# voletiv/mcvd-pytorch

Hardware: NVIDIA H100
Metric: frames/sec @100 DDPM steps, SMMNIST 64x64 (higher is better)
Workload: dtype f32 (fp16 hi/lo split on wgmma, fp32 accumulate)

## Files before the change

mcvd_b200/csrc/conv_umma.cu:

```cuda
#include <cuda.h>
#include <cuda_fp16.h>

#include <algorithm>
#include <cstring>

#include "mcvd_common.cuh"
#include "umma_ptx.cuh"

namespace mcvd {

constexpr int STAT_MT = 128;

namespace {

using namespace ptx;

constexpr int NPROD = 96;
constexpr int W_LOAD = 3;
constexpr int W_CONS = 4;
constexpr int NT_MAX3 = 192;
constexpr int REG_PROD3 = 96, REG_CONS3 = 136;
constexpr float STAT_SCALE = 65536.0f;
constexpr int TAB_NB = 8;
constexpr int HP_MAX = 512;
constexpr int PPT = (HP_MAX + NPROD - 1) / NPROD;
constexpr int RAW_STAGES = 2;
constexpr int MAX_RESIDENT = 12;

struct ConvMaps {
  CUtensorMap src[4];
  CUtensorMap tab;
};

struct ConvArgs {
  const float* s0;
  const float* s1;
  const float* s2;
  const float* s3;
  int C2, C3, nKB0;
  const __half* wpk;
  const float* bias;
  const float* res;
  const float* tab;
  int tab_planar;
  float* dst;
  unsigned long long* stats;
  int NJ;
  int B, H, W, C0, C1, Cout;
  int ks;
  int Wp, Pimg;
  int Qtot;
  int KB;
  int HP;
  int boxn, nbox;
  int raw_off, raw_stage, tab_off;
  int RA;
  int halo0;
  int nKB;
  int NB;
  int SA;
  int NPI;
  int tiles_n, ntiles;
  int act_in, act_out;
  int split;
  int tab_nb;
  float wscale, oscale;
};

__device__ __forceinline__ int decode_pos(const ConvArgs& a, int q, int& b_out) {
  if (q < 0 || q >= a.Qtot) return -1;
  const int b = q / a.Pimg;
  const int r = q - b * a.Pimg;
  const int rr = r / a.Wp, cc = r - rr * a.Wp;
  b_out = b;
  if (a.ks == 3) {
    if (rr == 0 || cc == 0) return -1;
    return (b * a.H + (rr - 1)) * a.W + (cc - 1);
  }
  return (b * a.H + rr) * a.W + cc;
}

__device__ __forceinline__ int first_raw(const ConvArgs& a, int q) {
  q = max(q, 0);
  if (q >= a.Qtot) return a.B * a.H * a.W;
  if (a.ks == 1) return q;
  const int b = q / a.Pimg;
  const int r = q - b * a.Pimg;
  const int rr = r / a.Wp, cc = r - rr * a.Wp;
  if (rr == 0) return b * a.H * a.W;
  return (b * a.H + (rr - 1)) * a.W + (cc == 0 ? 0 : cc - 1);
}

template <int NT, int NWG>
__global__ void __launch_bounds__(128 * (NWG + 1), 1) k_conv_umma(const ConvArgs a,
                                                                  const __grid_constant__ ConvMaps maps) {
  static_assert(NWG == 2 || (NWG == 3 && NT <= NT_MAX3), "three consumer warpgroups hold at most 96 accumulators");
  constexpr int MT = 64 * NWG;
  constexpr int NTHREADS = 128 * (NWG + 1);
  constexpr int NCONS = 4 * NWG;
  extern __shared__ __align__(1024) uint8_t smem_raw[];
  const int chunks = a.KB / 8;
  const uint32_t a_half_bytes = (uint32_t)chunks * a.HP * 16;
  const uint32_t a_stage_bytes = 2 * a_half_bytes;
  constexpr uint32_t b_step_bytes = 64u * NT;
  const uint32_t b_stage_bytes = (uint32_t)(a.KB / 16) * b_step_bytes;
  uint8_t* a_base = smem_raw;
  uint8_t* b_base = a_base + (size_t)a.SA * a_stage_bytes;
  uint8_t* raw_base = smem_raw + a.raw_off;
  int* pinfo = reinterpret_cast<int*>(raw_base + (size_t)a.RA * a.raw_stage);
  unsigned long long* stat_s = reinterpret_cast<unsigned long long*>(pinfo + PPT * NPROD);
  uint64_t* bars = reinterpret_cast<uint64_t*>(stat_s + (a.stats ? a.NJ * 2 * NT : 0));
  const uint32_t bar0 = smem_u32(bars);
  auto A_FULL = [&](int i) { return bar0 + 8u * i; };
  auto A_EMPTY = [&](int i) { return bar0 + 8u * (a.SA + i); };
  auto B_FULL = [&](int i) { return bar0 + 8u * (2 * a.SA + i); };
  auto B_EMPTY = [&](int i) { return bar0 + 8u * (2 * a.SA + a.NB + i); };
  auto R_FULL = [&](int i) { return bar0 + 8u * (2 * a.SA + 2 * a.NB + i); };
  const int groups_n = a.tiles_n / a.NPI;

  const int tid = threadIdx.x, warp = tid >> 5, lane = tid & 31;
  const int taps = a.ks * a.ks;

  if (tid == 0) {
    for (int i = 0; i < a.SA; ++i) { mbar_init(A_FULL(i), NPROD); mbar_init(A_EMPTY(i), NCONS); }
    for (int i = 0; i < a.NB; ++i) { mbar_init(B_FULL(i), 1); mbar_init(B_EMPTY(i), NCONS); }
    for (int i = 0; i < a.RA; ++i) mbar_init(R_FULL(i), 1);
    fence_barrier_init();
  }
  if (a.stats)
    for (int i = tid; i < a.NJ * 2 * NT; i += NTHREADS) stat_s[i] = 0ull;
  __syncthreads();

  if (warp < W_CONS) {
    if constexpr (NWG == 3) setmaxnreg_dec<REG_PROD3>();
    if (warp < W_LOAD) {
      const bool has_tab = a.tab != nullptr;
      const int ch = (lane >> 3) % chunks;
      const int ppass = NPROD / chunks;
      const int pp = warp * (32 / chunks) + (lane & 7) + 8 * ((lane >> 3) / chunks);
      const uint32_t rowb = (uint32_t)a.KB * 4, smask = a.KB == 32 ? 7u : 3u;
      auto tile_b0_of = [&](int t) {
        const int q_first = (t / groups_n) * MT - a.halo0;
        return q_first <= 0 ? 0 : min(a.B - 1, q_first / a.Pimg);
      };
      const uint32_t raw0 = smem_u32(raw_base);
      const uint32_t main_bytes = (uint32_t)a.nbox * a.boxn * rowb, ctr_bytes = (uint32_t)MT * rowb;
      const uint32_t tab_bytes = (uint32_t)a.tab_nb * a.KB * (a.tab_planar ? 12 : 16);
      int it = blockIdx.x, ikb = 0, ig = 0;
      auto issue_next = [&]() {
        if (it >= a.ntiles) return;
        const int p0 = (it / groups_n) * MT;
        const bool seg2 = ikb >= a.nKB0;
        int si, cc0;
        if (!seg2) {
          const int c0 = ikb * a.KB;
          if (c0 < a.C0) { si = 0; cc0 = c0; } else { si = 1; cc0 = c0 - a.C0; }
        } else {
          const int c0 = (ikb - a.nKB0) * a.KB;
          if (c0 < a.C2) { si = 2; cc0 = c0; } else { si = 3; cc0 = c0 - a.C2; }
        }
        const bool use_tab = has_tab && !seg2;
        const uint32_t dst = raw0 + (uint32_t)(ig % a.RA) * a.raw_stage;
        const uint32_t bar = R_FULL(ig % a.RA);
        mbar_arrive_expect_tx(bar, (seg2 ? ctr_bytes : main_bytes) + (use_tab ? tab_bytes : 0u));
        if (seg2) {
          tma_load_2d(dst, &maps.src[si], cc0, first_raw(a, p0), bar);
        } else {
          const int r0 = first_raw(a, p0 - a.halo0);
          for (int i = 0; i < a.nbox; ++i)
            tma_load_2d(dst + (uint32_t)i * a.boxn * rowb, &maps.src[si], cc0, r0 + i * a.boxn, bar);
        }
        if (use_tab) {
          if (a.tab_planar) tma_load_3d(dst + a.tab_off, &maps.tab, ikb * a.KB, 0, tile_b0_of(it), bar);
          else tma_load_2d(dst + a.tab_off, &maps.tab, 4 * ikb * a.KB, tile_b0_of(it), bar);
        }
        ++ig;
        if (++ikb == a.nKB) { ikb = 0; it += gridDim.x; }
      };
      if (tid == 0)
        for (int i = 0; i < a.RA - 1; ++i) issue_next();
      int g = 0;
      for (int t = blockIdx.x; t < a.ntiles; t += gridDim.x) {
        const int p0 = (t / groups_n) * MT;
        const int tb0 = tile_b0_of(t);
        const int raw_m = first_raw(a, p0 - a.halo0), raw_c = first_raw(a, p0);
        named_bar_sync(1, NPROD);
        for (int h = tid; h < a.HP; h += NPROD) {
          int b = tb0;
          const int pix = decode_pos(a, p0 - a.halo0 + h, b);
          pinfo[h] = pix < 0 ? -1 : ((b - tb0) << 16) | (pix - raw_m);
        }
        for (int kb = 0; kb < a.nKB; ++kb, ++g) {
          const int st = g % a.SA;
          const bool seg2 = kb >= a.nKB0;
          const bool use_tab = has_tab && !seg2;
          const int h_lo = seg2 ? a.halo0 : 0, h_hi = seg2 ? a.halo0 + MT : a.HP;
          const int roff = seg2 ? raw_c - raw_m : 0;
          named_bar_sync(1, NPROD);
          if (tid == 0) issue_next();
// ... 55 lines not shown
              hv = make_uint4(hw[0], hw[1], hw[2], hw[3]);
              lv = make_uint4(lw[0], lw[1], lw[2], lw[3]);
            }
            *reinterpret_cast<uint4*>(hi_base + (size_t)h * 16) = hv;
            *reinterpret_cast<uint4*>(lo_base + (size_t)h * 16) = lv;
          }
          fence_proxy_async();
          mbar_arrive(A_FULL(st));
        }
      }
    } else if (warp == W_LOAD) {
      if (elect_one()) {
        const uint32_t b0 = smem_u32(b_base);
        const int per_tile = a.nKB0 * taps + (a.nKB - a.nKB0);
        int st = 0, ph = 1;
        for (int t = blockIdx.x; t < a.ntiles; t += gridDim.x)
         for (int j = 0; j < a.NPI; ++j) {
          const int nt = (t % groups_n) * a.NPI + j;
          const uint8_t* wsrc = reinterpret_cast<const uint8_t*>(a.wpk) + (size_t)nt * per_tile * b_stage_bytes;
          for (int i = 0; i < per_tile; ++i) {
            mbar_wait(B_EMPTY(st), ph);
            mbar_arrive_expect_tx(B_FULL(st), b_stage_bytes);
            bulk_g2s(b0 + (uint32_t)st * b_stage_bytes, wsrc + (size_t)i * b_stage_bytes, b_stage_bytes, B_FULL(st));
            if (++st == a.NB) { st = 0; ph ^= 1; }
          }
        }
      }
      __syncwarp();
    }
  } else {
    if constexpr (NWG == 3) setmaxnreg_inc<REG_CONS3>();
    const int wg = (warp - W_CONS) >> 2;
    const int wq = (warp - W_CONS) & 3;
    const int ksteps = a.KB / 16;
    const uint32_t a_lbo = (uint32_t)a.HP * 16;
    const uint64_t a_proto = make_desc(0, a_lbo, 128), b_proto = make_desc(0, NT * 16, 128);
    const uint32_t a_half16 = a_half_bytes >> 4, b_lo16 = 2u * NT;
    const uint32_t a0_16 = smem_u32(a_base) >> 4, b0_16 = smem_u32(b_base) >> 4;
    const uint32_t a_stage16 = a_stage_bytes >> 4, b_stage16 = b_stage_bytes >> 4;
    const uint32_t a_lbo16 = a_lbo >> 4;
    int bst = 0, bph = 0, g0 = 0;
    for (int t = blockIdx.x; t < a.ntiles; t += gridDim.x, g0 += a.nKB)
     for (int j = 0; j < a.NPI; ++j) {
      const int p0 = (t / groups_n) * MT;
      const int n0 = ((t % groups_n) * a.NPI + j) * NT;
      const bool last_n = j == a.NPI - 1;
      float acc[NT / 2];
#pragma unroll
      for (int i = 0; i < NT / 2; ++i) acc[i] = 0.f;
      int pend_b = -1, pend_a = -1;
      for (int kb = 0; kb < a.nKB; ++kb) {
        const int g = g0 + kb;
        const int st = g % a.SA;
        mbar_wait(A_FULL(st), (g / a.SA) & 1);
        const uint32_t a_hi16 = a0_16 + (uint32_t)st * a_stage16 + (uint32_t)(a.halo0 + 64 * wg);
        const int ntap = (kb < a.nKB0) ? taps : 1;
        for (int tap = 0; tap < ntap; ++tap) {
          mbar_wait(B_FULL(bst), bph);
          const int shift = (a.ks == 3 && kb < a.nKB0) ? ((tap / 3 - 1) * a.Wp + (tap % 3 - 1)) : 0;
          const uint32_t a_tap16 = a_hi16 + (uint32_t)shift;
// ... 13 lines not shown
          wgmma_wait<1>();
          if (pend_b >= 0 && lane == 0) mbar_arrive(B_EMPTY(pend_b));
          if (pend_a >= 0 && lane == 0) mbar_arrive(A_EMPTY(pend_a));
          pend_b = bst;
          pend_a = (tap == ntap - 1 && last_n) ? st : -1;
          if (++bst == a.NB) { bst = 0; bph ^= 1; }
        }
      }
      wgmma_wait<0>();
#pragma unroll
      for (int i = 0; i < NT / 2; ++i) reg_fence(acc[i]);
      if (lane == 0) { mbar_arrive(B_EMPTY(pend_b)); if (pend_a >= 0) mbar_arrive(A_EMPTY(pend_a)); }

      const int r0 = 64 * wg + 16 * wq + (lane >> 2);
      const int cq = 2 * (lane & 3);
      int pix[2], slot[2];
      const int tile_b0 = min(a.B - 1, p0 / a.Pimg);
#pragma unroll
      for (int i = 0; i < 2; ++i) {
        int b = 0;
        pix[i] = decode_pos(a, p0 + r0 + 8 * i, b);
        slot[i] = pix[i] >= 0 ? b - tile_b0 : -1;
      }
      unsigned jmask = 0;
      if (a.stats) {
#pragma unroll 1
        for (int jj = 0; jj < a.NJ; ++jj)
          if (__ballot_sync(0xffffffffu, slot[0] == jj || slot[1] == jj)) jmask |= 1u << jj;
      }
#pragma unroll
      for (int j = 0; j < NT / 8; ++j) {
        const int n = n0 + 8 * j + cq;
        const float2 bv = a.bias ? __ldg(reinterpret_cast<const float2*>(a.bias + n)) : make_float2(0.f, 0.f);
        float v[2][2];
#pragma unroll
        for (int i = 0; i < 2; ++i) {
          float2 rv = make_float2(0.f, 0.f);
          if (a.res && pix[i] >= 0) rv = __ldg(reinterpret_cast<const float2*>(a.res + (long long)pix[i] * a.Cout + n));
          float x0 = (acc[4 * j + 2 * i] * a.wscale + bv.x + rv.x) * a.oscale;
          float x1 = (acc[4 * j + 2 * i + 1] * a.wscale + bv.y + rv.y) * a.oscale;
          if (a.act_out) { x0 = silu_f(x0); x1 = silu_f(x1); }
          v[i][0] = x0; v[i][1] = x1;
          if (pix[i] >= 0) *reinterpret_cast<float2*>(a.dst + (long long)pix[i] * a.Cout + n) = make_float2(x0, x1);
        }
        if (a.stats) {
#pragma unroll 1
          for (int jj = 0; jj < a.NJ; ++jj) {
            if (!(jmask & (1u << jj))) continue;
#pragma unroll
            for (int e = 0; e < 2; ++e) {
              long long s1 = 0;
              unsigned long long s2 = 0;
#pragma unroll
              for (int i = 0; i < 2; ++i) {
                if (slot[i] == jj) {
                  const int xi = __float2int_rn(v[i][e] * STAT_SCALE);
                  s1 += xi;
                  s2 += (unsigned long long)((long long)xi * (long long)xi);
                }
              }
#pragma unroll
              for (int o = 4; o <= 16; o <<= 1) {
                s1 += __shfl_xor_sync(0xffffffffu, s1, o);
                s2 += __shfl_xor_sync(0xffffffffu, s2, o);
              }
              if (lane < 4) {
                unsigned long long* sp = stat_s + (size_t)jj * 2 * NT + 8 * j + cq + e;
                atomicAdd(sp, (unsigned long long)s1);
                atomicAdd(sp + NT, s2);
              }
            }
          }
        }
      }
      if (a.stats) {
        named_bar_sync(2, 32 * NCONS);
        const int et = tid - W_CONS * 32;
        unsigned long long* gp = a.stats + (size_t)(p0 / MT) * a.NJ * 2 * a.Cout;
        for (int i = et; i < a.NJ * 2 * NT; i += 32 * NCONS) {
          const int jp = i / NT, n = i - jp * NT;
          gp[(size_t)jp * a.Cout + n0 + n] = stat_s[i];
          stat_s[i] = 0ull;
        }
        named_bar_sync(2, 32 * NCONS);
      }
    }
  }
}

__global__ void k_pack_weights(const float* __restrict__ w, __half* __restrict__ out, int taps, int Cin, int Cout,
                               int NT, int KB, float scale, int stage_off, int per_unit) {
  const int ksteps = KB / 16, nKB = Cin / KB, nNT = Cout / NT;
  const long long total = (long long)nNT * nKB * taps * ksteps * 2 * NT * 8;
  for (long long i = (long long)blockIdx.x * blockDim.x + threadIdx.x; i < total;
       i += (long long)gridDim.x * blockDim.x) {
    int e = (int)(i % 8);
    long long t = i / 8;
    int n = (int)(t % NT); t /= NT;
    int j = (int)(t % 2); t /= 2;
// ... 24 lines not shown
  if (C2 + C3 > 0 && pick_kb(C2, C3) < kb) kb = pick_kb(C2, C3);
  return kb;
}

struct Plan {
  int HP, NB, NJ;
  int boxn, nbox, tab_nb;
  int raw_off, raw_stage, tab_off, RA;
  size_t smem;
};

constexpr size_t SMEM_LIMIT = 227 * 1024;

size_t round1024(size_t x) { return (x + 1023) & ~(size_t)1023; }

bool make_plan(int H, int W, int ks, int KB, int NT, bool stats, int SA, int MT, Plan& p) {
  const int Wp = ks == 3 ? W + 1 : W;
  const int Pimg = ks == 3 ? (H + 1) * (W + 1) : H * W;
  const int halo0 = ks == 3 ? Wp + 1 : 0;
  p.HP = (MT + 2 * halo0 + 7) & ~7;
  p.NJ = (MT - 1) / Pimg + 2;
  if (p.HP > HP_MAX) return false;
  p.nbox = p.HP > 256 ? 2 : 1;
  p.boxn = p.nbox == 1 ? p.HP : ((p.HP / 2 + 7) & ~7);
  p.tab_nb = std::min(p.HP / Pimg + 2, TAB_NB);
  p.tab_off = p.nbox * p.boxn * KB * 4;
  p.raw_stage = (int)round1024((size_t)p.tab_off + (size_t)p.tab_nb * KB * 16);
  const size_t a_stage = (size_t)2 * (KB / 8) * p.HP * 16;
  const size_t b_stage = (size_t)(KB / 16) * 64 * NT;
  const size_t stat_bytes = stats ? (size_t)p.NJ * 2 * NT * 8 : 0;
  const size_t pinfo_bytes = (size_t)PPT * NPROD * 4;
  size_t bar_bytes = 0, fixed = 0;
  for (p.RA = RAW_STAGES; p.RA >= 1; --p.RA) {
    bar_bytes = 8 * (2 * SA + 20 + p.RA);
    fixed = round1024(SA * a_stage) + (size_t)p.RA * p.raw_stage + pinfo_bytes + stat_bytes + bar_bytes;
    if (fixed + 2 * b_stage <= SMEM_LIMIT) break;
  }
  if (p.RA == 0) return false;
  p.NB = (int)((SMEM_LIMIT - fixed) / b_stage);
  if (p.NB > 10) p.NB = 10;
  p.raw_off = (int)round1024(SA * a_stage + (size_t)p.NB * b_stage);
  p.smem = (size_t)p.raw_off + (size_t)p.RA * p.raw_stage + pinfo_bytes + stat_bytes + bar_bytes;
  return p.smem <= SMEM_LIMIT;
}

// ... 46 lines not shown
    if (nwg == 3) return launch_nt<NT, 3>(a, m, smem, grid, s);
  return launch_nt<NT, 2>(a, m, smem, grid, s);
}

int launch_conv(const McvdOp& op, cudaStream_t s, bool planar) {
  const char* name = planar ? "CONV_UMMA2" : "CONV_UMMA";
  MCVD_CHECK(op.src0 && op.w && op.dst && (op.C1 == 0 || op.src1), "%s: null pointer", name);
  MCVD_CHECK(op.i0 == 1 || op.i0 == 3, "%s: kernel size %d unsupported", name, op.i0);
  ConvArgs a;
  a.s0 = (const float*)op.src0; a.s1 = (const float*)op.src1; a.wpk = (const __half*)op.w;
  a.s2 = (const float*)op.src2; a.s3 = (const float*)op.src3; a.C2 = op.src2 ? op.C2 : 0; a.C3 = op.src3 ? op.C3 : 0;
  a.bias = (const float*)op.bias; a.res = (const float*)op.aux0; a.tab = (const float*)op.aux1;
  a.tab_planar = planar ? 1 : 0;
  a.dst = (float*)op.dst;
  a.stats = (unsigned long long*)op.dst2;
  a.B = op.B; a.H = op.H; a.W = op.W; a.C0 = op.C0; a.C1 = op.C1; a.Cout = op.Cout; a.ks = op.i0;
  const int NT = op.i1;
  a.KB = conv_kb(op.C0, op.C1, a.C2, a.C3);
  MCVD_CHECK(a.KB != 0, "%s: input channels (%d,%d | %d,%d) must be multiples of 16", name, op.C0, op.C1, a.C2, a.C3);
  MCVD_CHECK(!planar || op.i2 == 0 || op.i2 == a.KB, "CONV_UMMA2: weights packed for K-block %d, the conv uses %d",
             op.i2, a.KB);
  MCVD_CHECK(NT >= 16 && NT <= 256 && NT % 16 == 0 && op.Cout % NT == 0, "%s: n tile %d invalid for Cout %d", name, NT,
             op.Cout);
  if (a.ks == 3) { a.Wp = op.W + 1; a.Pimg = (op.H + 1) * (op.W + 1); }
  else { a.Wp = op.W; a.Pimg = op.H * op.W; }
  MCVD_CHECK((long long)op.B * a.Pimg < (1LL << 31), "%s: too many pixels", name);
  a.Qtot = op.B * a.Pimg;
  MCVD_CHECK(!a.stats || a.Pimg >= 64, "%s: epilogue statistics need images of >= 64 positions", name);
  a.halo0 = (a.ks == 3) ? a.Wp + 1 : 0;
  a.nKB0 = (op.C0 + op.C1) / a.KB;
  a.nKB = a.nKB0 + (a.C2 + a.C3) / a.KB;
  a.tiles_n = op.Cout / NT;
  const long long tiles128 = (a.Qtot + STAT_MT - 1) / STAT_MT;
  int dev = 0, sms = 132;
  cudaGetDevice(&dev);
  cudaDeviceGetAttribute(&sms, cudaDevAttrMultiProcessorCount, dev);
  const int mode = planar ? 0 : op.i2;
  MCVD_CHECK(mode >= 0 && mode <= 2, "%s: work organisation %d", name, mode);
  Plan p;
  const bool can_stay = a.ks == 1 && a.nKB == a.nKB0 && a.tiles_n > 1 && a.nKB <= MAX_RESIDENT &&
                        make_plan(op.H, op.W, a.ks, a.KB, NT, a.stats != nullptr, a.nKB, STAT_MT, p);
  const bool stay = can_stay && (mode == 2 || (mode == 0 && 2 * tiles128 >= sms));
  const int sa_req = planar ? 0 : op.i5;
  MCVD_CHECK(sa_req == 0 || ((sa_req == 2 || sa_req == 3) && !stay), "%s: %d slab stages", name, sa_req);
  a.SA = stay ? a.nKB : (sa_req ? sa_req : 2);
  a.NPI = stay ? a.tiles_n : 1;
  const int mt_req = planar ? 0 : op.i4;
  MCVD_CHECK(mt_req == 0 || mt_req == 128 || mt_req == 192, "%s: tile height %d", name, mt_req);
  const bool can3 = !planar && NT <= NT_MAX3 && !stay && !a.stats &&
                    make_plan(op.H, op.W, a.ks, a.KB, NT, false, a.SA, 192, p) &&
                    (!a.tab || p.HP / a.Pimg + 2 <= TAB_NB);
  MCVD_CHECK(mt_req != 192 || can3, "%s: 192-position tiles need streaming, NT <= %d, no statistics and %dx%d to fit",
             name, NT_MAX3, op.H, op.W);
  auto last_positions = [&](int mt) {
    const long long items = (a.Qtot + mt - 1) / mt * a.tiles_n;
    return (items + sms - 1) / sms * mt;
  };
  const int MT = mt_req ? mt_req : (can3 && p.NB >= 3 && last_positions(192) <= last_positions(128) ? 192 : 128);
  long long tiles_m = (a.Qtot + MT - 1) / MT;
  if (planar) tiles_m = (tiles_m + 1) & ~1LL;
  MCVD_CHECK(make_plan(op.H, op.W, a.ks, a.KB, NT, a.stats != nullptr, a.SA, MT, p),
             "%s: tile does not fit shared memory (W=%d)", name, op.W);
  a.HP = p.HP; a.NB = p.NB; a.NJ = p.NJ;
  a.boxn = p.boxn; a.nbox = p.nbox; a.raw_off = p.raw_off; a.raw_stage = p.raw_stage; a.tab_off = p.tab_off;
  a.RA = p.RA;
  a.act_in = (op.flags & MCVD_F_ACT_IN) ? 1 : 0;
  a.act_out = (op.flags & MCVD_F_ACT_OUT) ? 1 : 0;
  a.wscale = op.f1; a.oscale = op.f0;
  a.split = (op.i3 >= 1 && op.i3 <= 3) ? op.i3 : (op.i3 == 4 ? 0 : 3);
  {
    const int nb = a.HP / a.Pimg + 2;
    MCVD_CHECK(nb <= TAB_NB || !a.tab, "%s: %dx%d images are too small for the fused-norm path", name, op.H, op.W);
    a.tab_nb = (nb <= TAB_NB) ? nb : 0;
  }
  ConvMaps maps;
  memset(&maps, 0, sizeof(maps));
// ... 13 lines not shown
      const int Cin = op.C0 + op.C1;
      if (planar) {
        const cuuint64_t dims[3] = {(cuuint64_t)Cin, 3, (cuuint64_t)op.B};
        const cuuint64_t strides[2] = {(cuuint64_t)Cin * 4, (cuuint64_t)Cin * 12};
        const cuuint32_t box[3] = {(cuuint32_t)a.KB, 3, (cuuint32_t)a.tab_nb};
        if (encode_map(&maps.tab, a.tab, 3, dims, strides, box, CU_TENSOR_MAP_SWIZZLE_NONE, name)) return -1;
      } else {
        const cuuint64_t dims[2] = {(cuuint64_t)Cin * 4, (cuuint64_t)op.B};
        const cuuint64_t strides[1] = {(cuuint64_t)Cin * 16};
        const cuuint32_t box[2] = {(cuuint32_t)(4 * a.KB), (cuuint32_t)a.tab_nb};
        if (encode_map(&maps.tab, a.tab, 2, dims, strides, box, CU_TENSOR_MAP_SWIZZLE_NONE, name)) return -1;
      }
    }
  }
  MCVD_CHECK(tiles_m * a.tiles_n < (1LL << 31), "%s: too many tiles", name);
  a.ntiles = (int)(tiles_m * (a.tiles_n / a.NPI));
  const int grid = a.ntiles < sms ? a.ntiles : sms;
  switch (NT) {
#define MCVD_NT_CASE(n) case n: return launch_nt<n>(a, maps, p.smem, grid, MT / 64, s);
    MCVD_NT_CASE(16) MCVD_NT_CASE(32) MCVD_NT_CASE(48) MCVD_NT_CASE(64) MCVD_NT_CASE(80) MCVD_NT_CASE(96)
    MCVD_NT_CASE(112) MCVD_NT_CASE(128) MCVD_NT_CASE(144) MCVD_NT_CASE(160) MCVD_NT_CASE(176) MCVD_NT_CASE(192)
    MCVD_NT_CASE(208) MCVD_NT_CASE(224) MCVD_NT_CASE(240) MCVD_NT_CASE(256)
#undef MCVD_NT_CASE
    default: break;
  }
  MCVD_CHECK(false, "%s: n tile %d", name, NT);
}

long long pack(const float* w_taps, int taps, int Cin, int Cout, int n_tile, int KB, void* out, int scale_log2,
               int stage_off, int per_unit, void* stream) {
  if ((KB != 16 && KB != 32) || Cin % KB || n_tile < 16 || n_tile % 16 || Cout % n_tile) {
// ... 25 lines not shown
int launch_conv_umma2(const McvdOp& op, cudaStream_t s) { return launch_conv(op, s, true); }

}

extern "C" int mcvd_umma_kblock(int C0, int C1) { return mcvd::pick_kb(C0, C1); }

extern "C" long long mcvd_umma_pack_weights(const float* w_taps, int taps, int Cin, int Cout, int n_tile, int KB,
                                            void* out, int scale_log2, void* stream) {
  return mcvd::pack(w_taps, taps, Cin, Cout, n_tile, KB, out, scale_log2, 0, KB ? (Cin / KB) * taps : 0, stream);
}

extern "C" int mcvd_umma2_plan(int H, int W, int ks, int C0, int C1, int C2, int C3, int n_tile, int stats) {
  const int kb = mcvd::conv_kb(C0, C1, C2, C3);
  mcvd::Plan p;
  if (!kb || n_tile < 16 || n_tile > 256 || n_tile % 16) return 0;
  return mcvd::make_plan(H, W, ks, kb, n_tile, stats != 0, 2, mcvd::STAT_MT, p) ? kb : 0;
}

extern "C" int mcvd_umma2_plan_info(int H, int W, int ks, int C0, int C1, int C2, int C3, int n_tile, int stats,
                                    int* out) {
  const int kb = mcvd_umma2_plan(H, W, ks, C0, C1, C2, C3, n_tile, stats);
  if (!kb || !out) return -1;
  mcvd::Plan p;
  mcvd::make_plan(H, W, ks, kb, n_tile, stats != 0, 2, mcvd::STAT_MT, p);
  out[0] = kb; out[1] = p.HP; out[2] = 2; out[3] = p.RA; out[4] = p.NB; out[5] = p.NJ; out[6] = 0;
  out[7] = (int)p.smem; out[8] = 1; out[9] = 1;
  return 0;
}

extern "C" long long mcvd_umma2_stats_bytes(int B, int H, int W, int ks, int Cout) {
  const long long pimg = ks == 3 ? (long long)(H + 1) * (W + 1) : (long long)H * W;
  const long long tiles = 2 * ((B * pimg + 2 * mcvd::STAT_MT - 1) / (2 * mcvd::STAT_MT));
  const long long nj = (mcvd::STAT_MT - 1) / pimg + 2;
  return tiles * nj * 2 * Cout * 8;
}

extern "C" long long mcvd_umma2_pack_weights(const float* w_taps, int taps, int Cin, int Cout, int n_tile, int KB,
                                             void* out, int scale_log2, int stage_off, int per_unit, void* stream) {
  return mcvd::pack(w_taps, taps, Cin, Cout, n_tile, KB, out, scale_log2, stage_off, per_unit, stream);
// ... 2 lines not shown
```

mcvd_b200/program.py:

```python
from __future__ import annotations

import contextlib
import math
import os
from typing import Dict, List, Optional, Tuple

import torch

from . import arch, lib
from .lib import McvdOp

INV_SQRT2 = float(1.0 / math.sqrt(2.0))
GN_PPC = 64
GN_MIN_CHUNKS = 32


def gn_chunks(hw: int) -> int:
    return max(1, min(hw // 8, max(hw // GN_PPC, GN_MIN_CHUNKS)))


class Src:

    def __init__(self, t0, c0, t1=None, c1=0):
        self.t0, self.c0, self.t1, self.c1 = t0, c0, t1, c1
# ... 69 lines not shown
        self.cache_dir = os.environ.get("MCVD_WEIGHT_CACHE") or None
        self.packs_computed = 0
        self.packs_loaded = 0
        self.programs: Dict[int, Program] = {}
        self.launches_last_forward = 0

    MAX_PROGRAMS = 3

    def _version(self):
        ps = [p.detach() for p in self.module.parameters()]
        ids = tuple((p.data_ptr(), tuple(p.shape)) for p in ps)
        with torch.no_grad():
            fp = torch.stack(list(torch._foreach_norm(ps, 2)) + list(torch._foreach_norm(ps, 1))).double()
        return ids, fp

    def invalidate(self):
        self.packed_version = None

    def _sd(self, key):
        return self._params[key]

    def _cache_path(self):
        if not self.cache_dir or self.backend is not None or self.packed_version is None:
            return None
        import hashlib
        ids, fp = self.packed_version
        h = hashlib.sha256()
        h.update(repr((lib.ABI_VERSION, self.conv_mode, self.split_mode, [sh for _, sh in ids])).encode())
        h.update(fp.detach().cpu().numpy().tobytes())
        return os.path.join(self.cache_dir, f"mcvd_b200_packed_{h.hexdigest()[:32]}.pt")
# ... 180 lines not shown
            o = McvdOp()
            o.kind = kind
            o.B = B
            for k, v in kw.items():
                if k in ("src0", "src1", "w", "bias", "aux0", "aux1", "aux2", "dst", "dst2", "src2", "src3"):
                    if isinstance(v, torch.Tensor):
                        v = v.data_ptr()
                    setattr(o, k, v)
                else:
                    setattr(o, k, v)
            ops.append(o)
            return o

        sd = self._sd
        step, cnd = P.step_ops, P.cond_ops

        def conv(ops, key, src: Src, H: int, cout: int, ks: int, wname: str, bname: str, residual=None,
                 scale=1.0, tab=None, act_in=False, act_out=False, nin=False, wcat=None, bcat=None, shortcut=None,
                 stats=False):
            if wcat is not None:
                taps, bias = wcat, bcat
            elif nin:
                taps = sd(wname).float().unsqueeze(0).contiguous()
                bias = sd(bname).float().contiguous()
            else:
                taps = self._conv_taps(sd(wname))
                bias = sd(bname).float().contiguous()
            keep(bias)
            dst = f32(B, H, H, cout)
            nt = _pick_nt(cout) if cout % 16 == 0 else 0
# ... 52 lines not shown
                    else:
                        self.packed[pk] = self._pack_umma_fused(taps, sc[1], nt, kb)
                wp, wscale = self.packed[pk]
                nacc = 0
                fl = (lib.F_ACT_IN if act_in else 0) | (lib.F_ACT_OUT if act_out else 0)
                kw2 = {}
                if sc is not None:
                    kw2 = dict(src2=sc[0].t0, src3=sc[0].t1, C2=sc[0].c0, C3=sc[0].c1)
                st = None
                pimg = (H + 1) * (H + 1) if ks == 3 else H * H
                if stats and pimg >= 64 and self.epilogue_stats:
                    st = keep(torch.zeros(lib.umma2_stats_bytes(B, H, H, ks, cout) // 8, device=dev, dtype=torch.int64))
                    stats_of[dst.data_ptr()] = (st, ks)
                emit(ops, lib.OP_CONV_UMMA, H=H, W=H, C0=src.c0, C1=src.c1, Cout=cout, i0=ks, i1=nt, i2=nacc,
                     i3=self.split_mode, f0=scale, f1=wscale, src0=src.t0, src1=src.t1, w=wp, bias=bias, aux0=residual, aux1=tab,
                     dst=dst, dst2=st, flags=fl, **kw2)
                P.n_umma += 1
                return dst
            if tab is not None:
                a = f32(B, H, H, src.C)
                emit(ops, lib.OP_APPLY, H=H, W=H, C0=src.c0, C1=src.c1, src0=src.t0, src1=src.t1, aux0=tab, dst=a,
                     flags=lib.F_ACT_OUT if act_in else 0)
                src = Src(a, src.C)
            pk = (key, "simt")
            if pk not in self.packed:
                self.packed[pk] = self._pack_simt(taps)
            wp, coutp = self.packed[pk]
            emit(ops, lib.OP_CONV_SIMT, H=H, W=H, C0=src.c0, C1=src.c1, Cout=cout, i0=ks, i1=coutp, f0=scale,
                 src0=src.t0, src1=src.t1, w=wp, bias=bias, aux0=residual, dst=dst,
                 flags=lib.F_ACT_OUT if act_out else 0)
            P.n_simt += 1
# ... 290 lines not shown
            if torch.is_tensor(t):
                self.set_uniform_t(P, False)
                P.t.copy_(t.reshape(-1).to(torch.float32))
            else:
                self.set_uniform_t(P, True)
                P.t.fill_(float(t))
        if cond is not None and P.cond_in is not None:
            P.cond_in.copy_(cond.reshape(P.cond_in.shape))

    def forward(self, x, y, cond=None):
        ns = self.spec
        B = x.shape[0]
        if ns.cond_ch > 0 and cond is None:
            raise RuntimeError("mcvd_b200: this network was built with conditioning frames; cond is required")
        with self._devctx():
            P = self.program(B)
            self.set_inputs(P, x.float(), y, cond.float() if cond is not None else None)
            self.run_cond(P)
            self.run_step(P)
            self._run(P.out_arr, 1)
            self.launches_last_forward = P.cond_launches + P.step_launches + 1
            return P.out.clone()
```

mcvd_b200/samplers.py:

```python
from __future__ import annotations

import logging
import math
from typing import List, Optional

import numpy as np
import torch

from . import lib
from .model import UNetMore_DDPM


def _unwrap(scorenet) -> UNetMore_DDPM:
    net = scorenet.module if hasattr(scorenet, "module") else scorenet
    if not isinstance(net, UNetMore_DDPM):
        raise TypeError("mcvd_b200 samplers drive mcvd_b200.UNetMore_DDPM modules "
                        f"(got {type(net).__name__}); use the reference samplers for reference modules")
    return net


def _schedule(net, subsample_steps):
    alphas, alphas_prev, betas = net.alphas.detach().cpu(), net.alphas_prev.detach().cpu(), net.betas.detach().cpu()
    steps = np.arange(len(betas))
    if subsample_steps is not None and subsample_steps < len(alphas):
# ... 30 lines not shown
    dev = torch.device(device) if device is not None else torch.device("cuda", torch.cuda.current_device())
    if dev.type != "cuda":
        raise RuntimeError("mcvd_b200.samplers.gamma_noise draws on CUDA devices only (no CPU fallback)")
    B, C, H, W = shape
    out = torch.empty(tuple(shape), device=dev, dtype=torch.float32)
    if out.numel() == 0:
        return out
    op = lib.McvdOp()
    op.kind, op.flags, op.B, op.H, op.W, op.C0 = lib.OP_NOISE, lib.F_GAMMA, B, H, W, C
    op.i0, op.i1, op.i2, op.i3 = int(seed & 0x7FFFFFFF), int((seed >> 31) & 0x7FFFFFFF), int(clip0), int(step)
    op.f5, op.f6, op.f7 = float(scale), float(k), float(theta)
    op.dst = out.data_ptr()
    with torch.cuda.device(dev):
        lib.run_program(lib.make_ops([op]), 1, torch.cuda.current_stream(dev).cuda_stream)
    return out


class _Loop:

    def __init__(self, x_mod, scorenet, cond):
        self.net = _unwrap(scorenet)
        self.eng = self.net.engine()
        self.dev = self.eng.device
        self.out_dev = x_mod.device
        self.B = x_mod.shape[0]
        self.shape = x_mod.shape
        self.launches = 0
        if self.eng.spec.cond_ch > 0 and cond is None:
            raise RuntimeError("mcvd_b200: cond is required by this network")
        self._ctx = self.eng._devctx()
# ... 57 lines not shown
    if verbose:
        print(msg)
    if log:
        logging.info(msg)


def _warm_start(lp, alpha, warm_noise, gamma, philox_seed, clip_offset, i):
    if warm_noise is None and gamma is not None:
        lp.update(0.0, 0.0, 0.0, alpha.sqrt().item(), 0.0, (1 - alpha).sqrt().item(), False,
                  philox=(philox_seed, clip_offset), step=GAMMA_WARM_STEP + i, gamma=gamma)
        return
    z0 = warm_noise if warm_noise is not None else torch.randn(lp.P.noise.shape, device=lp.dev)
    lp.update(0.0, 0.0, 0.0, alpha.sqrt().item(), 0.0, (1 - alpha).sqrt().item(), False, noise=z0)


@torch.no_grad()
def ddpm_sampler(x_mod, scorenet, cond=None, just_beta=False, final_only=False, denoise=True, subsample_steps=None,
                 same_noise=False, noise_val=None, frac_steps=None, verbose=False, log=False, clip_before=True,
                 t_min=-1, gamma=False, noise_list: Optional[List[torch.Tensor]] = None, philox_seed=None,
                 clip_offset=0, warm_noise: Optional[torch.Tensor] = None, **kwargs):
    t_min = -1 if t_min is None else t_min
    if gamma and philox_seed is None:
        philox_seed = draw_seed()
    lp = _Loop(x_mod, scorenet, cond)
    try:
        steps, alphas, alphas_prev, betas = _schedule(lp.net, subsample_steps)
        if gamma:
            ks_cum, thetas = _gamma_schedule(lp.net, subsample_steps)
        if frac_steps is not None:
            steps = steps[int((1 - frac_steps) * len(steps)):]
# ... 45 lines not shown
                          philox=None if philox_seed is None or noise is not None else (philox_seed, clip_offset),
                          step=i, gamma=gp(i))
        if denoise:
            lp.eps(float(L - 1))
            lp.update(0.0, 0.0, 0.0, 1.0, -(1 - alphas[-1]).sqrt().item(), 0.0, False)
            if not final_only:
                images.append(lp.state().to("cpu"))
        ddpm_sampler.last_launches = lp.launches
        if final_only:
            return lp.result(lp.state().unsqueeze(0))
        return torch.stack(images)
    finally:
        lp.close()


@torch.no_grad()
def ddim_sampler(x_mod, scorenet, cond=None, final_only=False, denoise=True, subsample_steps=None, verbose=False,
                 log=True, clip_before=True, t_min=-1, gamma=False, warm_noise: Optional[torch.Tensor] = None,
                 philox_seed=None, clip_offset=0, **kwargs):
    t_min = -1 if t_min is None else t_min
    if gamma and philox_seed is None:
        philox_seed = draw_seed()
    lp = _Loop(x_mod, scorenet, cond)
    try:
        steps, alphas, alphas_prev, betas = _schedule(lp.net, subsample_steps)
        if gamma:
            ks_cum, thetas = _gamma_schedule(lp.net, subsample_steps)
        gp = (lambda j: _gamma_params(ks_cum, thetas, alphas, j)) if gamma else (lambda j: None)
        L = len(steps)
        images = []
# ... 12 lines not shown
                images.append(lp.state().to("cpu"))
            if (verbose or log) and (i == 0 or (i + 1) % max(L // 10, 1) == 0):
                _log_line("DDIM gamma" if gamma else "DDIM", i, L, lp.eps_nchw(), lp.state(), c_alpha, verbose, log)
        if denoise:
            lp.eps(float(L - 1))
            lp.update(0.0, 0.0, 0.0, 1.0, -(1 - alphas[-1]).sqrt().item(), 0.0, False)
            if not final_only:
                images.append(lp.state().to("cpu"))
        if final_only:
            return lp.result(lp.state().unsqueeze(0))
        return torch.stack(images)
    finally:
        lp.close()


@torch.no_grad()
def FPNDM_sampler(x_mod, scorenet, cond=None, final_only=False, denoise=True, subsample_steps=None, verbose=False,
                  log=True, clip_before=True, t_min=-1, gamma=False, **kwargs):
    lp = _Loop(x_mod, scorenet, cond)
    try:
        net = lp.net
        alphas = net.alphas.detach().cpu()
        alphas_old = alphas.flip(0)
        skip = len(alphas) // subsample_steps
        steps = list(range(0, len(alphas), skip))
        steps_next = [-1] + steps[:-1]
        P = lp.P

        def eps_at(x, t):
            lp.eng.set_inputs(P, x=x)
# ... 52 lines not shown
```

Measured before the change: 138.6.

## Allow 192-row conv tiles with epilogue GroupNorm stats via paired tiles and 32-bit limbs

Convolutions that also accumulate GroupNorm statistics can now use the three-warpgroup 192-position tile. Each unit processes two consecutive M tiles so the statistics stay aligned to 128-position blocks, using double-buffered shared accumulators. The 64-bit shared atomics are replaced by 32-bit atomics on five 24-bit limbs, and a range flag triggers a fallback rerun when an output falls outside the representable range. This adds more atomics, more shared memory, a host-side flag check after each forward or sampler call, and a possible full rerun.

```diff
diff --git a/mcvd_b200/csrc/conv_umma.cu b/mcvd_b200/csrc/conv_umma.cu
--- a/mcvd_b200/csrc/conv_umma.cu
+++ b/mcvd_b200/csrc/conv_umma.cu
@@ -19,8 +19,10 @@
 constexpr int W_LOAD = 3;
 constexpr int W_CONS = 4;
 constexpr int NT_MAX3 = 192;
-constexpr int REG_PROD3 = 96, REG_CONS3 = 136;
+constexpr int REG_PROD3 = 104, REG_CONS3 = 136;
 constexpr float STAT_SCALE = 65536.0f;
+constexpr float STAT_RANGE = 4096.0f;
+constexpr int STAT_LIMBS = 5;
 constexpr int TAB_NB = 8;
 constexpr int HP_MAX = 512;
 constexpr int PPT = (HP_MAX + NPROD - 1) / NPROD;
@@ -45,6 +47,7 @@
   int tab_planar;
   float* dst;
   unsigned long long* stats;
+  unsigned* range_flag;
   int NJ;
   int B, H, W, C0, C1, Cout;
   int ks;
@@ -60,7 +63,8 @@
   int NB;
   int SA;
   int NPI;
-  int tiles_n, ntiles;
+  int MP;
+  int tiles_m, tiles_n, ntiles;
   int act_in, act_out;
   int split;
   int tab_nb;
@@ -89,6 +93,18 @@
   const int rr = r / a.Wp, cc = r - rr * a.Wp;
   if (rr == 0) return b * a.H * a.W;
   return (b * a.H + (rr - 1)) * a.W + (cc == 0 ? 0 : cc - 1);
+}
+
+__device__ __forceinline__ int unit_of(const ConvArgs& a, int w) { return a.MP == 2 ? w >> 1 : w; }
+
+__device__ __forceinline__ int m_tile_of(const ConvArgs& a, int groups_n, int w) {
+  const int u = unit_of(a, w);
+  return (u / groups_n) * a.MP + (w - u * a.MP);
+}
+
+__device__ __forceinline__ int next_item(const ConvArgs& a, int groups_n, int w) {
+  const int u = unit_of(a, w), h = w - u * a.MP;
+  return h + 1 < a.MP && (u / groups_n) * a.MP + h + 1 < a.tiles_m ? w + 1 : (u + (int)gridDim.x) * a.MP;
 }
 
 template <int NT, int NWG>
@@ -108,8 +124,9 @@
   uint8_t* b_base = a_base + (size_t)a.SA * a_stage_bytes;
   uint8_t* raw_base = smem_raw + a.raw_off;
   int* pinfo = reinterpret_cast<int*>(raw_base + (size_t)a.RA * a.raw_stage);
-  unsigned long long* stat_s = reinterpret_cast<unsigned long long*>(pinfo + PPT * NPROD);
-  uint64_t* bars = reinterpret_cast<uint64_t*>(stat_s + (a.stats ? a.NJ * 2 * NT : 0));
+  unsigned* stat_s = reinterpret_cast<unsigned*>(pinfo + PPT * NPROD);
+  const int stat_buf = a.NJ * STAT_LIMBS * NT;
+  uint64_t* bars = reinterpret_cast<uint64_t*>(stat_s + (a.stats ? ((a.MP * stat_buf + 1) & ~1) : 0));
   const uint32_t bar0 = smem_u32(bars);
   auto A_FULL = [&](int i) { return bar0 + 8u * i; };
   auto A_EMPTY = [&](int i) { return bar0 + 8u * (a.SA + i); };
@@ -128,7 +145,7 @@
     fence_barrier_init();
   }
   if (a.stats)
-    for (int i = tid; i < a.NJ * 2 * NT; i += NTHREADS) stat_s[i] = 0ull;
+    for (int i = tid; i < a.MP * stat_buf; i += NTHREADS) stat_s[i] = 0u;
   __syncthreads();
 
   if (warp < W_CONS) {
@@ -139,17 +156,17 @@
       const int ppass = NPROD / chunks;
       const int pp = warp * (32 / chunks) + (lane & 7) + 8 * ((lane >> 3) / chunks);
       const uint32_t rowb = (uint32_t)a.KB * 4, smask = a.KB == 32 ? 7u : 3u;
-      auto tile_b0_of = [&](int t) {
-        const int q_first = (t / groups_n) * MT - a.halo0;
+      auto tile_b0_of = [&](int p0) {
+        const int q_first = p0 - a.halo0;
         return q_first <= 0 ? 0 : min(a.B - 1, q_first / a.Pimg);
       };
       const uint32_t raw0 = smem_u32(raw_base);
       const uint32_t main_bytes = (uint32_t)a.nbox * a.boxn * rowb, ctr_bytes = (uint32_t)MT * rowb;
       const uint32_t tab_bytes = (uint32_t)a.tab_nb * a.KB * (a.tab_planar ? 12 : 16);
-      int it = blockIdx.x, ikb = 0, ig = 0;
+      int iw = blockIdx.x * a.MP, ikb = 0, ig = 0;
       auto issue_next = [&]() {
-        if (it >= a.ntiles) return;
-        const int p0 = (it / groups_n) * MT;
+        if (unit_of(a, iw) >= a.ntiles) return;
+        const int p0 = m_tile_of(a, groups_n, iw) * MT;
         const bool seg2 = ikb >= a.nKB0;
         int si, cc0;
         if (!seg2) {
@@ -171,18 +188,18 @@
             tma_load_2d(dst + (uint32_t)i * a.boxn * rowb, &maps.src[si], cc0, r0 + i * a.boxn, bar);
         }
         if (use_tab) {
-          if (a.tab_planar) tma_load_3d(dst + a.tab_off, &maps.tab, ikb * a.KB, 0, tile_b0_of(it), bar);
-          else tma_load_2d(dst + a.tab_off, &maps.tab, 4 * ikb * a.KB, tile_b0_of(it), bar);
+          if (a.tab_planar) tma_load_3d(dst + a.tab_off, &maps.tab, ikb * a.KB, 0, tile_b0_of(p0), bar);
+          else tma_load_2d(dst + a.tab_off, &maps.tab, 4 * ikb * a.KB, tile_b0_of(p0), bar);
         }
         ++ig;
-        if (++ikb == a.nKB) { ikb = 0; it += gridDim.x; }
+        if (++ikb == a.nKB) { ikb = 0; iw = next_item(a, groups_n, iw); }
       };
       if (tid == 0)
         for (int i = 0; i < a.RA - 1; ++i) issue_next();
       int g = 0;
-      for (int t = blockIdx.x; t < a.ntiles; t += gridDim.x) {
-        const int p0 = (t / groups_n) * MT;
-        const int tb0 = tile_b0_of(t);
+      for (int w = blockIdx.x * a.MP; unit_of(a, w) < a.ntiles; w = next_item(a, groups_n, w)) {
+        const int p0 = m_tile_of(a, groups_n, w) * MT;
+        const int tb0 = tile_b0_of(p0);
         const int raw_m = first_raw(a, p0 - a.halo0), raw_c = first_raw(a, p0);
         named_bar_sync(1, NPROD);
         for (int h = tid; h < a.HP; h += NPROD) {
@@ -268,9 +285,9 @@
         const uint32_t b0 = smem_u32(b_base);
         const int per_tile = a.nKB0 * taps + (a.nKB - a.nKB0);
         int st = 0, ph = 1;
-        for (int t = blockIdx.x; t < a.ntiles; t += gridDim.x)
+        for (int w = blockIdx.x * a.MP; unit_of(a, w) < a.ntiles; w = next_item(a, groups_n, w))
          for (int j = 0; j < a.NPI; ++j) {
-          const int nt = (t % groups_n) * a.NPI + j;
+          const int nt = (unit_of(a, w) % groups_n) * a.NPI + j;
           const uint8_t* wsrc = reinterpret_cast<const uint8_t*>(a.wpk) + (size_t)nt * per_tile * b_stage_bytes;
           for (int i = 0; i < per_tile; ++i) {
             mbar_wait(B_EMPTY(st), ph);
@@ -294,10 +311,12 @@
     const uint32_t a_stage16 = a_stage_bytes >> 4, b_stage16 = b_stage_bytes >> 4;
     const uint32_t a_lbo16 = a_lbo >> 4;
     int bst = 0, bph = 0, g0 = 0;
-    for (int t = blockIdx.x; t < a.ntiles; t += gridDim.x, g0 += a.nKB)
+    for (int w = blockIdx.x * a.MP; unit_of(a, w) < a.ntiles; w = next_item(a, groups_n, w), g0 += a.nKB)
      for (int j = 0; j < a.NPI; ++j) {
-      const int p0 = (t / groups_n) * MT;
-      const int n0 = ((t % groups_n) * a.NPI + j) * NT;
+      const int u = unit_of(a, w), h = w - u * a.MP;
+      const int mt = m_tile_of(a, groups_n, w);
+      const int p0 = mt * MT;
+      const int n0 = ((u % groups_n) * a.NPI + j) * NT;
       const bool last_n = j == a.NPI - 1;
       float acc[NT / 2];
 #pragma unroll
@@ -341,15 +360,19 @@
 
       const int r0 = 64 * wg + 16 * wq + (lane >> 2);
       const int cq = 2 * (lane & 3);
+      const int su0 = (mt - h) * MT / STAT_MT;
+      const int sk = (p0 + 64 * wg) / STAT_MT;
+      unsigned* sbuf = stat_s + ((sk - su0) & 1) * stat_buf;
       int pix[2], slot[2];
-      const int tile_b0 = min(a.B - 1, p0 / a.Pimg);
+      const int stat_b0 = min(a.B - 1, sk * STAT_MT / a.Pimg);
 #pragma unroll
       for (int i = 0; i < 2; ++i) {
         int b = 0;
         pix[i] = decode_pos(a, p0 + r0 + 8 * i, b);
-        slot[i] = pix[i] >= 0 ? b - tile_b0 : -1;
+        slot[i] = pix[i] >= 0 ? b - stat_b0 : -1;
       }
       unsigned jmask = 0;
+      bool out_of_range = false;
       if (a.stats) {
 #pragma unroll 1
         for (int jj = 0; jj < a.NJ; ++jj)
@@ -372,44 +395,69 @@
         }
         if (a.stats) {
 #pragma unroll 1
-          for (int jj = 0; jj < a.NJ; ++jj) {
-            if (!(jmask & (1u << jj))) continue;
-#pragma unroll
-            for (int e = 0; e < 2; ++e) {
-              long long s1 = 0;
-              unsigned long long s2 = 0;
-#pragma unroll
-              for (int i = 0; i < 2; ++i) {
-                if (slot[i] == jj) {
+          for (unsigned jm = jmask; jm; jm &= jm - 1) {
+            const int jj = __ffs(jm) - 1;
+            long long s1[2] = {0, 0};
+            unsigned long long s2[2] = {0ull, 0ull};
+#pragma unroll
+            for (int i = 0; i < 2; ++i) {
+              if (slot[i] == jj) {
+#pragma unroll
+                for (int e = 0; e < 2; ++e) {
+                  out_of_range |= !(fabsf(v[i][e]) <= STAT_RANGE);
                   const int xi = __float2int_rn(v[i][e] * STAT_SCALE);
-                  s1 += xi;
-                  s2 += (unsigned long long)((long long)xi * (long long)xi);
+                  s1[e] += xi;
+                  s2[e] += (unsigned long long)((long long)xi * (long long)xi);
                 }
               }
-#pragma unroll
-              for (int o = 4; o <= 16; o <<= 1) {
-                s1 += __shfl_xor_sync(0xffffffffu, s1, o);
-                s2 += __shfl_xor_sync(0xffffffffu, s2, o);
-              }
-              if (lane < 4) {
-                unsigned long long* sp = stat_s + (size_t)jj * 2 * NT + 8 * j + cq + e;
-                atomicAdd(sp, (unsigned long long)s1);
-                atomicAdd(sp + NT, s2);
-              }
+            }
+            const int ce = (lane >> 2) & 1;
+            long long t1 = ce ? s1[1] : s1[0];
+            unsigned long long t2 = ce ? s2[1] : s2[0];
+            t1 += __shfl_xor_sync(0xffffffffu, ce ? s1[0] : s1[1], 4);
+            t2 += __shfl_xor_sync(0xffffffffu, ce ? s2[0] : s2[1], 4);
+#pragma unroll
+            for (int o = 8; o <= 16; o <<= 1) {
+              t1 += __shfl_xor_sync(0xffffffffu, t1, o);
+              t2 += __shfl_xor_sync(0xffffffffu, t2, o);
+            }
+            if (lane < 8) {
+              unsigned* sp = sbuf + (size_t)jj * STAT_LIMBS * NT + 8 * j + cq + ce;
+              atomicAdd(sp, (unsigned)t1 & 0xffffffu);
+              atomicAdd(sp + NT, (unsigned)(t1 >> 24));
+              atomicAdd(sp + 2 * NT, (unsigned)t2 & 0xffffffu);
+              atomicAdd(sp + 3 * NT, (unsigned)(t2 >> 24) & 0xffffffu);
+              atomicAdd(sp + 4 * NT, (unsigned)(t2 >> 48));
             }
           }
         }
       }
       if (a.stats) {
         named_bar_sync(2, 32 * NCONS);
+        const bool last = h + 1 == a.MP || mt + 1 == a.tiles_m;
+        const int lo = h * MT / STAT_MT, hi = last ? ((h + 1) * MT + STAT_MT - 1) / STAT_MT : (h + 1) * MT / STAT_MT;
+        const int stat_tiles = MT == STAT_MT ? a.tiles_m : (a.Qtot + STAT_MT - 1) / STAT_MT;
         const int et = tid - W_CONS * 32;
-        unsigned long long* gp = a.stats + (size_t)(p0 / MT) * a.NJ * 2 * a.Cout;
-        for (int i = et; i < a.NJ * 2 * NT; i += 32 * NCONS) {
-          const int jp = i / NT, n = i - jp * NT;
-          gp[(size_t)jp * a.Cout + n0 + n] = stat_s[i];
-          stat_s[i] = 0ull;
+        for (int l = lo; l < hi; ++l) {
+          unsigned* buf = stat_s + (l & 1) * stat_buf;
+          unsigned long long* gp = a.stats + (size_t)(su0 + l) * a.NJ * 2 * a.Cout;
+          const bool write = su0 + l < stat_tiles;
+          for (int i = et; i < a.NJ * NT; i += 32 * NCONS) {
+            const int jj = i / NT, n = i - jj * NT;
+            unsigned* sp = buf + (size_t)jj * STAT_LIMBS * NT + n;
+            if (write) {
+              const long long s1 = (long long)sp[0] + (long long)(int)sp[NT] * (1LL << 24);
+              const unsigned long long s2 = (unsigned long long)sp[2 * NT] + ((unsigned long long)sp[3 * NT] << 24) +
+                                            ((unsigned long long)sp[4 * NT] << 48);
+              gp[(size_t)(2 * jj) * a.Cout + n0 + n] = (unsigned long long)s1;
+              gp[(size_t)(2 * jj + 1) * a.Cout + n0 + n] = s2;
+            }
+#pragma unroll
+            for (int k = 0; k < STAT_LIMBS; ++k) sp[k * NT] = 0u;
+          }
         }
         named_bar_sync(2, 32 * NCONS);
+        if (out_of_range && a.range_flag) *a.range_flag = 1u;
       }
     }
   }
@@ -464,12 +512,12 @@
 
 size_t round1024(size_t x) { return (x + 1023) & ~(size_t)1023; }
 
-bool make_plan(int H, int W, int ks, int KB, int NT, bool stats, int SA, int MT, Plan& p) {
+bool make_plan(int H, int W, int ks, int KB, int NT, int stat_bufs, int SA, int MT, Plan& p) {
   const int Wp = ks == 3 ? W + 1 : W;
   const int Pimg = ks == 3 ? (H + 1) * (W + 1) : H * W;
   const int halo0 = ks == 3 ? Wp + 1 : 0;
   p.HP = (MT + 2 * halo0 + 7) & ~7;
-  p.NJ = (MT - 1) / Pimg + 2;
+  p.NJ = (STAT_MT - 1) / Pimg + 2;
   if (p.HP > HP_MAX) return false;
   p.nbox = p.HP > 256 ? 2 : 1;
   p.boxn = p.nbox == 1 ? p.HP : ((p.HP / 2 + 7) & ~7);
@@ -478,7 +526,7 @@
   p.raw_stage = (int)round1024((size_t)p.tab_off + (size_t)p.tab_nb * KB * 16);
   const size_t a_stage = (size_t)2 * (KB / 8) * p.HP * 16;
   const size_t b_stage = (size_t)(KB / 16) * 64 * NT;
-  const size_t stat_bytes = stats ? (size_t)p.NJ * 2 * NT * 8 : 0;
+  const size_t stat_bytes = (size_t)((stat_bufs * p.NJ * STAT_LIMBS * NT + 1) & ~1) * 4;
   const size_t pinfo_bytes = (size_t)PPT * NPROD * 4;
   size_t bar_bytes = 0, fixed = 0;
   for (p.RA = RAW_STAGES; p.RA >= 1; --p.RA) {
@@ -555,6 +603,7 @@
   a.tab_planar = planar ? 1 : 0;
   a.dst = (float*)op.dst;
   a.stats = (unsigned long long*)op.dst2;
+  a.range_flag = a.stats ? (unsigned*)op.aux2 : nullptr;
   a.B = op.B; a.H = op.H; a.W = op.W; a.C0 = op.C0; a.C1 = op.C1; a.Cout = op.Cout; a.ks = op.i0;
   const int NT = op.i1;
   a.KB = conv_kb(op.C0, op.C1, a.C2, a.C3);
@@ -580,7 +629,7 @@
   MCVD_CHECK(mode >= 0 && mode <= 2, "%s: work organisation %d", name, mode);
   Plan p;
   const bool can_stay = a.ks == 1 && a.nKB == a.nKB0 && a.tiles_n > 1 && a.nKB <= MAX_RESIDENT &&
-                        make_plan(op.H, op.W, a.ks, a.KB, NT, a.stats != nullptr, a.nKB, STAT_MT, p);
+                        make_plan(op.H, op.W, a.ks, a.KB, NT, a.stats ? 1 : 0, a.nKB, STAT_MT, p);
   const bool stay = can_stay && (mode == 2 || (mode == 0 && 2 * tiles128 >= sms));
   const int sa_req = planar ? 0 : op.i5;
   MCVD_CHECK(sa_req == 0 || ((sa_req == 2 || sa_req == 3) && !stay), "%s: %d slab stages", name, sa_req);
@@ -588,19 +637,22 @@
   a.NPI = stay ? a.tiles_n : 1;
   const int mt_req = planar ? 0 : op.i4;
   MCVD_CHECK(mt_req == 0 || mt_req == 128 || mt_req == 192, "%s: tile height %d", name, mt_req);
-  const bool can3 = !planar && NT <= NT_MAX3 && !stay && !a.stats &&
-                    make_plan(op.H, op.W, a.ks, a.KB, NT, false, a.SA, 192, p) &&
+  const int mp3 = a.stats ? 2 : 1;
+  const bool can3 = !planar && NT <= NT_MAX3 && !stay &&
+                    make_plan(op.H, op.W, a.ks, a.KB, NT, a.stats ? mp3 : 0, a.SA, 192, p) &&
                     (!a.tab || p.HP / a.Pimg + 2 <= TAB_NB);
-  MCVD_CHECK(mt_req != 192 || can3, "%s: 192-position tiles need streaming, NT <= %d, no statistics and %dx%d to fit",
-             name, NT_MAX3, op.H, op.W);
-  auto last_positions = [&](int mt) {
-    const long long items = (a.Qtot + mt - 1) / mt * a.tiles_n;
-    return (items + sms - 1) / sms * mt;
+  MCVD_CHECK(mt_req != 192 || can3, "%s: 192-position tiles need streaming, NT <= %d and %dx%d to fit", name, NT_MAX3,
+             op.H, op.W);
+  auto last_positions = [&](int mt, int mp) {
+    const long long units = ((a.Qtot + mt - 1) / mt + mp - 1) / mp * a.tiles_n;
+    return (units + sms - 1) / sms * mt * mp;
   };
-  const int MT = mt_req ? mt_req : (can3 && p.NB >= 3 && last_positions(192) <= last_positions(128) ? 192 : 128);
+  const int MT = mt_req ? mt_req
+                        : (can3 && p.NB >= 3 && last_positions(192, mp3) <= last_positions(128, 1) ? 192 : 128);
+  a.MP = MT == 192 ? mp3 : 1;
   long long tiles_m = (a.Qtot + MT - 1) / MT;
   if (planar) tiles_m = (tiles_m + 1) & ~1LL;
-  MCVD_CHECK(make_plan(op.H, op.W, a.ks, a.KB, NT, a.stats != nullptr, a.SA, MT, p),
+  MCVD_CHECK(make_plan(op.H, op.W, a.ks, a.KB, NT, a.stats ? a.MP : 0, a.SA, MT, p),
              "%s: tile does not fit shared memory (W=%d)", name, op.W);
   a.HP = p.HP; a.NB = p.NB; a.NJ = p.NJ;
   a.boxn = p.boxn; a.nbox = p.nbox; a.raw_off = p.raw_off; a.raw_stage = p.raw_stage; a.tab_off = p.tab_off;
@@ -644,7 +696,8 @@
     }
   }
   MCVD_CHECK(tiles_m * a.tiles_n < (1LL << 31), "%s: too many tiles", name);
-  a.ntiles = (int)(tiles_m * (a.tiles_n / a.NPI));
+  a.tiles_m = (int)tiles_m;
+  a.ntiles = (int)((tiles_m + a.MP - 1) / a.MP * (a.tiles_n / a.NPI));
   const int grid = a.ntiles < sms ? a.ntiles : sms;
   switch (NT) {
 #define MCVD_NT_CASE(n) case n: return launch_nt<n>(a, maps, p.smem, grid, MT / 64, s);
@@ -700,7 +753,7 @@
   const int kb = mcvd::conv_kb(C0, C1, C2, C3);
   mcvd::Plan p;
   if (!kb || n_tile < 16 || n_tile > 256 || n_tile % 16) return 0;
-  return mcvd::make_plan(H, W, ks, kb, n_tile, stats != 0, 2, mcvd::STAT_MT, p) ? kb : 0;
+  return mcvd::make_plan(H, W, ks, kb, n_tile, stats != 0 ? 1 : 0, 2, mcvd::STAT_MT, p) ? kb : 0;
 }
 
 extern "C" int mcvd_umma2_plan_info(int H, int W, int ks, int C0, int C1, int C2, int C3, int n_tile, int stats,
@@ -708,7 +761,7 @@
   const int kb = mcvd_umma2_plan(H, W, ks, C0, C1, C2, C3, n_tile, stats);
   if (!kb || !out) return -1;
   mcvd::Plan p;
-  mcvd::make_plan(H, W, ks, kb, n_tile, stats != 0, 2, mcvd::STAT_MT, p);
+  mcvd::make_plan(H, W, ks, kb, n_tile, stats != 0 ? 1 : 0, 2, mcvd::STAT_MT, p);
   out[0] = kb; out[1] = p.HP; out[2] = 2; out[3] = p.RA; out[4] = p.NB; out[5] = p.NJ; out[6] = 0;
   out[7] = (int)p.smem; out[8] = 1; out[9] = 1;
   return 0;
diff --git a/mcvd_b200/program.py b/mcvd_b200/program.py
--- a/mcvd_b200/program.py
+++ b/mcvd_b200/program.py
@@ -3,6 +3,7 @@
 import contextlib
 import math
 import os
+import warnings
 from typing import Dict, List, Optional, Tuple
 
 import torch
@@ -107,6 +108,15 @@
             fp = torch.stack(list(torch._foreach_norm(ps, 2)) + list(torch._foreach_norm(ps, 1))).double()
         return ids, fp
 
+    def check_stats_range(self) -> bool:
+        if not self.epilogue_stats or not any(int(P.stats_flag.item()) for P in self.programs.values()):
+            return True
+        warnings.warn("mcvd_b200: a conv output exceeded |x| <= 2^12, the range of the epilogue GroupNorm statistics; "
+                      "rerunning with the GroupNorm partial pass (MCVD_EPISTATS=0) from now on", RuntimeWarning)
+        self.epilogue_stats = False
+        self.programs = {}
+        return False
+
     def invalidate(self):
         self.packed_version = None
 
@@ -317,6 +327,7 @@
 
         sd = self._sd
         step, cnd = P.step_ops, P.cond_ops
+        P.stats_flag = keep(torch.zeros(1, device=dev, dtype=torch.int32))
 
         def conv(ops, key, src: Src, H: int, cout: int, ks: int, wname: str, bname: str, residual=None,
                  scale=1.0, tab=None, act_in=False, act_out=False, nin=False, wcat=None, bcat=None, shortcut=None,
@@ -399,7 +410,7 @@
                     stats_of[dst.data_ptr()] = (st, ks)
                 emit(ops, lib.OP_CONV_UMMA, H=H, W=H, C0=src.c0, C1=src.c1, Cout=cout, i0=ks, i1=nt, i2=nacc,
                      i3=self.split_mode, f0=scale, f1=wscale, src0=src.t0, src1=src.t1, w=wp, bias=bias, aux0=residual, aux1=tab,
-                     dst=dst, dst2=st, flags=fl, **kw2)
+                     aux2=P.stats_flag if st is not None else None, dst=dst, dst2=st, flags=fl, **kw2)
                 P.n_umma += 1
                 return dst
             if tab is not None:
@@ -720,10 +731,13 @@
         if ns.cond_ch > 0 and cond is None:
             raise RuntimeError("mcvd_b200: this network was built with conditioning frames; cond is required")
         with self._devctx():
-            P = self.program(B)
-            self.set_inputs(P, x.float(), y, cond.float() if cond is not None else None)
-            self.run_cond(P)
-            self.run_step(P)
-            self._run(P.out_arr, 1)
+            while True:
+                P = self.program(B)
+                self.set_inputs(P, x.float(), y, cond.float() if cond is not None else None)
+                self.run_cond(P)
+                self.run_step(P)
+                self._run(P.out_arr, 1)
+                if self.check_stats_range():
+                    break
             self.launches_last_forward = P.cond_launches + P.step_launches + 1
             return P.out.clone()
diff --git a/mcvd_b200/samplers.py b/mcvd_b200/samplers.py
--- a/mcvd_b200/samplers.py
+++ b/mcvd_b200/samplers.py
@@ -1,5 +1,6 @@
 from __future__ import annotations
 
+import functools
 import logging
 import math
 from typing import List, Optional
@@ -68,6 +69,22 @@
     with torch.cuda.device(dev):
         lib.run_program(lib.make_ops([op]), 1, torch.cuda.current_stream(dev).cuda_stream)
     return out
+
+
+def _stats_range_guard(sampler):
+    @functools.wraps(sampler)
+    def run(x_mod, scorenet, *args, **kwargs):
+        eng = _unwrap(scorenet).engine()
+        cuda_dev = eng.device if eng.device.type == "cuda" else None
+        rng = (torch.random.get_rng_state(), torch.cuda.get_rng_state(cuda_dev) if cuda_dev is not None else None)
+        out = sampler(x_mod, scorenet, *args, **kwargs)
+        if not eng.check_stats_range():
+            torch.random.set_rng_state(rng[0])
+            if cuda_dev is not None:
+                torch.cuda.set_rng_state(rng[1], cuda_dev)
+            out = sampler(x_mod, scorenet, *args, **kwargs)
+        return out
+    return run
 
 
 class _Loop:
@@ -155,6 +172,7 @@
     lp.update(0.0, 0.0, 0.0, alpha.sqrt().item(), 0.0, (1 - alpha).sqrt().item(), False, noise=z0)
 
 
+@_stats_range_guard
 @torch.no_grad()
 def ddpm_sampler(x_mod, scorenet, cond=None, just_beta=False, final_only=False, denoise=True, subsample_steps=None,
                  same_noise=False, noise_val=None, frac_steps=None, verbose=False, log=False, clip_before=True,
@@ -230,6 +248,7 @@
         lp.close()
 
 
+@_stats_range_guard
 @torch.no_grad()
 def ddim_sampler(x_mod, scorenet, cond=None, final_only=False, denoise=True, subsample_steps=None, verbose=False,
                  log=True, clip_before=True, t_min=-1, gamma=False, warm_noise: Optional[torch.Tensor] = None,
@@ -272,6 +291,7 @@
         lp.close()
 
 
+@_stats_range_guard
 @torch.no_grad()
 def FPNDM_sampler(x_mod, scorenet, cond=None, final_only=False, denoise=True, subsample_steps=None, verbose=False,
                   log=True, clip_before=True, t_min=-1, gamma=False, **kwargs):
```

New measurement: 138.1, median of 6. No clear change (-0.4%).
